# stanford-iprl-lab/nerf_shared

Measured on AMD Instinct MI355X. Metric: rays_per_sec, higher is better.
Workload: dtype bf16; 1 GPU; lego_halfres_400x400_64c+128f_viewdirs_8x256_chunk4096; entry=Renderer.render(c2w=pose, retraw=False), chunk=4096, N_samples=64, N_importance=128, weights=random-init seeds 0/10, parallelism=single GPU

## Files before the change

### nerf_shared_amd/csrc/capi.hip

```cpp
#include <hip/hip_runtime.h>

#include <atomic>
#include <cmath>

#include <cstdio>
#include <cstring>
#include <mutex>
#include <utility>
#include <new>
#include <string>
#include <vector>

#include "kernels.h"
#include "program.h"

using namespace na;

namespace {
thread_local std::string g_err;

std::string lds_msg(const char *what, size_t bytes) {
    return std::string(what) + ": the per-ray scratch needs " + std::to_string(bytes) + " bytes of LDS per workgroup, the CU has " +
           std::to_string(LDS_LIMIT_BYTES) + " (fewer samples per ray)";
}
// ... 654 lines not shown
    if (Ni > 0 && !io->u && !io->t_lin_imp) return fail(NERF_AMD_EINVAL, "need u or t_lin_imp for sample_pdf");
    const nerf_amd_model *fm = fine ? fine : coarse;
    const int och = coarse->prog.out_ch;
    if (Ni > 0 && fm->prog.out_ch != och) return fail(NERF_AMD_EINVAL, "coarse and fine models disagree on output channels");
    if (och < 4) return fail(NERF_AMD_EINVAL, "field must output at least 4 channels");
    const bool has_vd = io->ray_ch > 8;
    if ((coarse->prog.arch.use_viewdirs != 0) != has_vd || (fm->prog.arch.use_viewdirs != 0) != has_vd)
        return fail(NERF_AMD_EINVAL, "ray batch width does not match the models' use_viewdirs");
    if (io->workspace_bytes < nerf_amd_render_rays_workspace(cfg, R, och) || !io->workspace)
        return fail(NERF_AMD_EINVAL, "workspace too small");
    p->cfg = cfg; p->coarse = coarse; p->fm = fm; p->io = io; p->R = R;
    p->Nc = Nc; p->Ni = Ni; p->Nf = Nf; p->och = och; p->has_vd = has_vd;

    char *w = static_cast<char *>(io->workspace);
    auto take = [&](size_t bytes) { float *q = reinterpret_cast<float *>(w); w += align_up(bytes); return q; };
    p->z_c = take(R * Nc * sizeof(float));
    p->raw_c = take(R * Nc * och * sizeof(float));
    p->w_c = take(R * Nc * sizeof(float));
    p->z_f = p->raw_f = nullptr;
    if (Ni > 0) {
        p->z_f = take(R * (size_t)Nf * sizeof(float));
        p->raw_f = take(R * (size_t)Nf * och * sizeof(float));
        if (io->z_vals) p->z_f = io->z_vals;
        if (io->raw) p->raw_f = io->raw;
    } else {
        if (io->z_vals) p->z_c = io->z_vals;
        if (io->raw) p->raw_c = io->raw;
        if (io->weights) p->w_c = io->weights;
    }
    return NERF_AMD_OK;
}

int stage_z(ChunkPlan &p, hipStream_t s) {
    const nerf_amd_render_io *io = p.io;
    int rc = 0;
    if (io->z_coarse) {
        if (p.Ni == 0 && io->z_vals)
            rc = hipMemcpyAsync(io->z_vals, io->z_coarse, p.R * p.Nc * sizeof(float), hipMemcpyDeviceToDevice, s) == hipSuccess
                     ? 0 : NERF_AMD_EHIP;
        else
            p.z_c = const_cast<float *>(io->z_coarse);
    } else {
        rc = launch_coarse_z(io->rays, io->ray_ch, io->t_vals, p.cfg->perturb ? io->t_rand : nullptr, p.R, p.Nc,
                             p.cfg->lindisp, p.cfg->perturb, p.z_c, s);
    }
    return rc ? fail(rc, "coarse_z launch failed") : NERF_AMD_OK;
}

int stage_field(const ChunkPlan &p, bool fine_pass, hipStream_t s) {
    MlpArgs a;
    std::memset(&a, 0, sizeof(a));
    a.rays = p.io->rays; a.ray_stride = p.io->ray_ch;
    a.viewdirs = p.has_vd ? p.io->rays + 8 : nullptr; a.vd_stride = p.io->ray_ch;
    if (!fine_pass) {
        a.z_vals = p.z_c; a.P = p.R * p.Nc; a.S = p.Nc; a.out = p.raw_c;
        return run_field(p.coarse, a, p.cfg->precision, s);
    }
    a.z_vals = p.z_f; a.P = p.R * (int64_t)p.Nf; a.S = p.Nf; a.out = p.raw_f;
    return run_field(p.fm, a, p.cfg->precision, s);
}

CompositeJob final_job(const ChunkPlan &p) {
    const nerf_amd_render_io *io = p.io;
    CompositeJob j;
    std::memset(&j, 0, sizeof(j));
    const bool two_pass = p.Ni > 0;
    j.raw = two_pass ? p.raw_f : p.raw_c; j.raw_ch = p.och; j.z = two_pass ? p.z_f : p.z_c;
    j.rays_d = io->rays + 3; j.rays_d_stride = io->ray_ch;
    j.noise = p.cfg->use_noise ? (two_pass ? io->noise1 : io->noise0) : nullptr;
    j.R = p.R; j.S = two_pass ? p.Nf : p.Nc; j.white_bkgd = p.cfg->white_bkgd;
    j.rgb = io->rgb_map; j.disp = io->disp_map; j.acc = io->acc_map; j.weights = two_pass ? io->weights : p.w_c;
    return j;
}

int stage_final(const ChunkPlan &p, hipStream_t s) {
    const CompositeJob j = final_job(p);
    int rc = launch_composite(j.raw, j.raw_ch, j.z, j.rays_d, j.rays_d_stride, j.noise, j.R, j.S, j.white_bkgd, j.rgb, j.disp,
                              j.acc, j.weights, nullptr, s);
    return rc ? fail(rc, "composite launch failed") : NERF_AMD_OK;
}

int stage_mid(const ChunkPlan &p, const ChunkPlan *prev, hipStream_t s) {
    const nerf_amd_render_io *io = p.io;
    CompositeJob cj;
    std::memset(&cj, 0, sizeof(cj));
    cj.raw = p.raw_c; cj.raw_ch = p.och; cj.z = p.z_c; cj.rays_d = io->rays + 3; cj.rays_d_stride = io->ray_ch;
    cj.noise = p.cfg->use_noise ? io->noise0 : nullptr; cj.R = p.R; cj.S = p.Nc; cj.white_bkgd = p.cfg->white_bkgd;
    cj.rgb = io->rgb0; cj.disp = io->disp0; cj.acc = io->acc0; cj.weights = nullptr;
    ResampleJob rj;
    std::memset(&rj, 0, sizeof(rj));
    rj.u = io->u; rj.t_lin = io->t_lin_imp; rj.Ni = p.Ni; rj.z_fine = p.z_f; rj.z_std = io->z_std;
    CompositeJob fj;
    if (prev) fj = final_job(*prev);
    int rc = launch_mid_stage(cj, rj, prev ? &fj : nullptr, s);
    if (rc == NERF_AMD_EINVAL && resample_lds_bytes(p.Nc, p.Ni, true) > LDS_LIMIT_BYTES)
        return fail(rc, lds_msg("render_rays (compositing + resampling)", resample_lds_bytes(p.Nc, p.Ni, true)));
    return rc ? fail(rc, "composite/resample launch failed") : NERF_AMD_OK;
}
}

extern "C" {

int nerf_amd_render_rays(const nerf_amd_render_cfg *cfg, const nerf_amd_model *coarse, const nerf_amd_model *fine,
                         const nerf_amd_render_io *io, int64_t R, void *stream) {
    if (R == 0 && cfg && coarse && io) return NERF_AMD_OK;
    ChunkPlan p;
    int rc = plan_chunk(cfg, coarse, fine, io, R, &p);
    if (rc) return rc;
    hipStream_t s = static_cast<hipStream_t>(stream);
    if ((rc = stage_z(p, s)) || (rc = stage_field(p, false, s))) return rc;
    if (p.Ni == 0) return stage_final(p, s);
    if ((rc = stage_mid(p, nullptr, s)) || (rc = stage_field(p, true, s))) return rc;
    return stage_final(p, s);
}

int nerf_amd_render_chunks(const nerf_amd_render_cfg *cfg, const nerf_amd_model *coarse, const nerf_amd_model *fine,
                           const nerf_amd_render_io *ios, const int64_t *R, int32_t n_chunks, void *stream) {
    if (n_chunks < 0 || (n_chunks > 0 && (!ios || !R))) return fail(NERF_AMD_EINVAL, "bad chunk list");
    hipStream_t s = static_cast<hipStream_t>(stream);
    std::vector<ChunkPlan> plans;
    plans.reserve(n_chunks);
    for (int i = 0; i < n_chunks; ++i) {
        if (R[i] <= 0) continue;
        ChunkPlan p;
        int rc = plan_chunk(cfg, coarse, fine, &ios[i], R[i], &p);
        if (rc) return rc;
        plans.push_back(p);
    }
    const int n = (int)plans.size();
    for (int i = 0; i + 1 < n; ++i)
        if (plans[i].io->workspace == plans[i + 1].io->workspace)
            return fail(NERF_AMD_EINVAL, "consecutive chunks must use distinct workspaces");
    int rc = 0;
    for (int k = 0; k < n && !rc; ++k) {
        ChunkPlan &p = plans[k];
        if ((rc = stage_z(p, s)) || (rc = stage_field(p, false, s))) break;
        if (p.Ni == 0) { rc = stage_final(p, s); continue; }
        if ((rc = stage_mid(p, k > 0 ? &plans[k - 1] : nullptr, s))) break;
        rc = stage_field(p, true, s);
    }
    if (!rc && n > 0 && plans[n - 1].Ni > 0) rc = stage_final(plans[n - 1], s);
    return rc;
}

}

namespace {
constexpr int64_t SUPER_CHUNK_RAYS = 32768;
constexpr int BATCH_SLOTS = 3;

struct SideLane {
    hipStream_t stream = nullptr;
    hipStream_t more[2] = {nullptr, nullptr};
    std::vector<hipEvent_t> free_events;
};
std::mutex g_lane_mu;
SideLane g_lanes[64];

}
namespace na {
namespace {
struct DeviceGuard {
    int prev = -1;
    bool switched = false;
    hipError_t err = hipSuccess;
    explicit DeviceGuard(int device) {
        err = hipGetDevice(&prev);
        if (err == hipSuccess && prev != device) {
            err = hipSetDevice(device);
            switched = err == hipSuccess;
        }
    }
    ~DeviceGuard() { if (switched) (void)hipSetDevice(prev); }
};
}

int lane_acquire(int device, int n_events, hipStream_t *side, std::vector<hipEvent_t> *events) {
    if (device < 0 || device >= 64) return fail(NERF_AMD_EINVAL, "device index out of range");
    std::lock_guard<std::mutex> lk(g_lane_mu);
    DeviceGuard guard(device);
    if (guard.err != hipSuccess) return hip_fail(guard.err, "hipSetDevice(lane device)");
    SideLane &l = g_lanes[device];
    if (!l.stream) HIP_TRY(hipStreamCreateWithFlags(&l.stream, hipStreamNonBlocking));
    *side = l.stream;
    events->clear();
    for (int i = 0; i < n_events; ++i) {
        hipEvent_t e;
        if (!l.free_events.empty()) { e = l.free_events.back(); l.free_events.pop_back(); }
        else if (hipError_t err = hipEventCreateWithFlags(&e, hipEventDisableTiming); err != hipSuccess) {
            for (hipEvent_t got : *events) l.free_events.push_back(got);
            events->clear();
            return hip_fail(err, "hipEventCreateWithFlags");
        }
        events->push_back(e);
    }
    return NERF_AMD_OK;
}
int lane_streams(int device, int n, hipStream_t *out) {
    if (device < 0 || device >= 64 || n < 1 || n > 3) return fail(NERF_AMD_EINVAL, "lane_streams: device or count out of range");
    std::lock_guard<std::mutex> lk(g_lane_mu);
    DeviceGuard guard(device);
    if (guard.err != hipSuccess) return hip_fail(guard.err, "hipSetDevice(lane device)");
    SideLane &l = g_lanes[device];
    if (!l.stream) HIP_TRY(hipStreamCreateWithFlags(&l.stream, hipStreamNonBlocking));
    out[0] = l.stream;
    for (int i = 1; i < n; ++i) {
        if (!l.more[i - 1]) HIP_TRY(hipStreamCreateWithFlags(&l.more[i - 1], hipStreamNonBlocking));
        out[i] = l.more[i - 1];
    }
    return NERF_AMD_OK;
}
void lane_release(int device, const std::vector<hipEvent_t> &events) {
    std::lock_guard<std::mutex> lk(g_lane_mu);
    for (hipEvent_t e : events) g_lanes[device].free_events.push_back(e);
}
}
namespace {

nerf_amd_render_io io_rows(const nerf_amd_render_cfg *cfg, const nerf_amd_render_io &io, int64_t r0, int och, void *ws, int64_t ws_bytes) {
    nerf_amd_render_io o = io;
    const int64_t Nc = cfg->N_samples, Ni = cfg->N_importance, Sl = Nc + Ni;
    auto f = [&](const float *p, int64_t row_floats) { return p ? p + r0 * row_floats : nullptr; };
    auto g = [&](float *p, int64_t row_floats) { return p ? p + r0 * row_floats : nullptr; };
    o.rays = f(io.rays, io.ray_ch);
    o.t_rand = f(io.t_rand, Nc); o.noise0 = f(io.noise0, Nc); o.noise1 = f(io.noise1, Sl);
    o.u = f(io.u, Ni); o.z_coarse = f(io.z_coarse, Nc);
    o.rgb_map = g(io.rgb_map, 3); o.disp_map = g(io.disp_map, 1); o.acc_map = g(io.acc_map, 1);
    o.rgb0 = g(io.rgb0, 3); o.disp0 = g(io.disp0, 1); o.acc0 = g(io.acc0, 1); o.z_std = g(io.z_std, 1);
    o.raw = g(io.raw, Sl * och); o.weights = g(io.weights, Sl); o.z_vals = g(io.z_vals, Sl);
    o.workspace = ws; o.workspace_bytes = ws_bytes;
    return o;
}

int64_t n_super_chunks(int64_t N) { return N <= SUPER_CHUNK_RAYS + SUPER_CHUNK_RAYS / 2 ? 1 : (N + SUPER_CHUNK_RAYS - 1) / SUPER_CHUNK_RAYS; }
}

extern "C" {

int64_t nerf_amd_render_batch_workspace(const nerf_amd_render_cfg *cfg, int64_t N, int32_t out_ch) {
    if (!cfg || N < 0) return -1;
    const int64_t n = n_super_chunks(N);
    const int64_t per = nerf_amd_render_rays_workspace(cfg, n == 1 ? N : SUPER_CHUNK_RAYS, out_ch);
    return per * (n < BATCH_SLOTS ? n : BATCH_SLOTS);
}

int nerf_amd_render_batch(const nerf_amd_render_cfg *cfg, const nerf_amd_model *coarse, const nerf_amd_model *fine,
                          const nerf_amd_render_io *io, int64_t N, void *stream) {
    if (!cfg || !coarse || !io || N < 0) return fail(NERF_AMD_EINVAL, "null argument");
    if (N == 0) return NERF_AMD_OK;
    const int64_t n = n_super_chunks(N);
    if (n == 1) return nerf_amd_render_rays(cfg, coarse, fine, io, N, stream);
    const int och = coarse->prog.out_ch;
    const int64_t per = nerf_amd_render_rays_workspace(cfg, SUPER_CHUNK_RAYS, och);
    const int slots = (int)(n < BATCH_SLOTS ? n : BATCH_SLOTS);
    if (!io->workspace || io->workspace_bytes < per * slots) return fail(NERF_AMD_EINVAL, "workspace too small (nerf_amd_render_batch_workspace)");
    if (!io->z_coarse && cfg->perturb && !io->t_rand) return fail(NERF_AMD_EINVAL, "perturb set but neither z_coarse nor t_rand given");

    std::vector<nerf_amd_render_io> ios((size_t)n);
    std::vector<ChunkPlan> plans((size_t)n);
    for (int64_t k = 0; k < n; ++k) {
        const int64_t r0 = k * SUPER_CHUNK_RAYS, R = (k + 1 == n) ? N - r0 : SUPER_CHUNK_RAYS;
        ios[k] = io_rows(cfg, *io, r0, och, static_cast<char *>(io->workspace) + (k % slots) * per, per);
        int rc = plan_chunk(cfg, coarse, fine, &ios[k], R, &plans[k]);
        if (rc) return rc;
    }
    hipStream_t main_s = static_cast<hipStream_t>(stream), side = nullptr;
    const int device = coarse->device;
    const bool two_pass = plans[0].Ni > 0;
    std::vector<hipEvent_t> ev;
    int rc = lane_acquire(device, (int)(3 * n + 1), &side, &ev);
    if (rc) return rc;
    hipEvent_t *ec = ev.data(), *em = ev.data() + n, *ef = ev.data() + 2 * n;
    hipEvent_t start = ev[3 * n];
    auto H = [&](hipError_t e, const char *what) { if (e != hipSuccess && !rc) rc = hip_fail(e, what); };
    H(hipEventRecord(start, main_s), "hipEventRecord");
    H(hipStreamWaitEvent(side, start, 0), "hipStreamWaitEvent");

    auto coarse_field = [&](int64_t k) {
        if (k >= slots) H(hipStreamWaitEvent(main_s, em[k - slots + (two_pass ? 1 : 0)], 0), "hipStreamWaitEvent");
        if (!rc) rc = stage_z(plans[k], main_s);
        if (!rc) rc = stage_field(plans[k], false, main_s);
        H(hipEventRecord(ec[k], main_s), "hipEventRecord");
    };
    if (two_pass) {
        hipStream_t fine_s = main_s;
        hipStream_t lanes2[2];
        if (g_variant == 44 && lane_streams(device, 2, lanes2) == NERF_AMD_OK) {
            fine_s = lanes2[1];
            H(hipStreamWaitEvent(fine_s, start, 0), "hipStreamWaitEvent");
        }
        coarse_field(0);
        for (int64_t k = 0; k < n && !rc; ++k) {
            if (k + 1 < n) coarse_field(k + 1);
            H(hipStreamWaitEvent(side, ec[k], 0), "hipStreamWaitEvent");
            if (k > 0) H(hipStreamWaitEvent(side, ef[k - 1], 0), "hipStreamWaitEvent");
            if (!rc) rc = stage_mid(plans[k], k > 0 ? &plans[k - 1] : nullptr, side);
            H(hipEventRecord(em[k], side), "hipEventRecord");
            H(hipStreamWaitEvent(fine_s, em[k], 0), "hipStreamWaitEvent");
            if (!rc) rc = stage_field(plans[k], true, fine_s);
            H(hipEventRecord(ef[k], fine_s), "hipEventRecord");
        }
        H(hipStreamWaitEvent(side, ef[n - 1], 0), "hipStreamWaitEvent");
        if (!rc) rc = stage_final(plans[n - 1], side);
    } else {
        for (int64_t k = 0; k < n && !rc; ++k) {
            coarse_field(k);
            H(hipStreamWaitEvent(side, ec[k], 0), "hipStreamWaitEvent");
            if (!rc) rc = stage_final(plans[k], side);
            H(hipEventRecord(em[k], side), "hipEventRecord");
        }
    }
    H(hipEventRecord(start, side), "hipEventRecord");
    H(hipStreamWaitEvent(main_s, start, 0), "hipStreamWaitEvent");
    lane_release(device, ev);
    return rc;
}

}

extern "C" {

int nerf_amd_set_tuning(int key, int value) {
    if (key == 0 && value >= 0 && value <= 115) { g_variant.store(value, std::memory_order_relaxed); return NERF_AMD_OK; }
    if (key == 1 && value >= 0 && value <= 1) { g_density_route.store(value, std::memory_order_relaxed); return NERF_AMD_OK; }
    return fail(NERF_AMD_EINVAL, "unknown tuning key/value");
}

int nerf_amd_profile_enable(int on) {
    std::lock_guard<std::mutex> lk(g_prof_mu);
    g_prof_on = on != 0;
    return NERF_AMD_OK;
}

int nerf_amd_profile_collect(int64_t launches[3], double total_ms[3], double total_points[3]) {
    std::lock_guard<std::mutex> lk(g_prof_mu);
    for (int c = 0; c < 3; ++c) { launches[c] = 0; total_ms[c] = 0.0; total_points[c] = 0.0; }
    for (const ProfRec &r : g_prof_recs) {
        float ms = 0.f;
        if (hipEventSynchronize(r.b) == hipSuccess && hipEventElapsedTime(&ms, r.a, r.b) == hipSuccess) {
            launches[r.cls] += 1; total_ms[r.cls] += ms; total_points[r.cls] += r.points;
        }
        g_prof_free.emplace_back(r.a, r.b);
    }
    g_prof_recs.clear();
    return NERF_AMD_OK;
}

int nerf_amd_get_rays_backward(int32_t H, int32_t W, const double *K4, int64_t pix0, int64_t n, const float *g_rays_o,
                               const float *g_rays_d, float *g_c2w, void *stream) {
    if (H < 1 || W < 1 || !K4 || pix0 < 0 || n < 0 || pix0 + n > (int64_t)H * W || !g_c2w)
        return fail(NERF_AMD_EINVAL, "bad get_rays_backward arguments");
    int rc = launch_get_rays_bwd(H, W, K4, pix0, n, g_rays_o, g_rays_d, g_c2w, static_cast<hipStream_t>(stream));
    return rc ? fail(rc, "get_rays backward launch failed") : NERF_AMD_OK;
}

int nerf_amd_img2mse(const float *x, const float *y, int64_t n, float *out, float *partials, void *stream) {
    if (n < 1 || !x || !y || !out) return fail(NERF_AMD_EINVAL, "bad img2mse arguments");
    int rc = na::launch_img2mse(x, y, n, out, partials, static_cast<hipStream_t>(stream));
    return rc ? fail(rc, rc == NERF_AMD_EINVAL ? "img2mse: n > 16384 needs the partials buffer" : "img2mse launch failed") : NERF_AMD_OK;
}

int nerf_amd_img2mse_backward(const float *x, const float *y, int64_t n, const float *g, float *gx, float *gy, void *stream) {
    if (n < 1 || !x || !y || !g) return fail(NERF_AMD_EINVAL, "bad img2mse_backward arguments");
    int rc = na::launch_img2mse_bwd(x, y, n, g, gx, gy, static_cast<hipStream_t>(stream));
    return rc ? fail(rc, "img2mse_backward launch failed") : NERF_AMD_OK;
}

int nerf_amd_assemble_rays(const float *rays_o, const float *rays_d, const float *viewdir_src, int64_t n, float near,
                           float far, float *out, void *stream) {
    if (n < 0 || (n > 0 && (!rays_o || !rays_d || !out))) return fail(NERF_AMD_EINVAL, "bad assemble_rays arguments");
    int rc = na::launch_assemble_rays(rays_o, rays_d, viewdir_src, n, near, far, out, static_cast<hipStream_t>(stream));
    return rc ? fail(rc, "assemble_rays launch failed") : NERF_AMD_OK;
}

int nerf_amd_adam_step(int32_t n, float *const *params, const float *const *grads, float *const *exp_avg,
                       float *const *exp_avg_sq, const int64_t *numel, int64_t step, double lr, double beta1,
                       double beta2, double eps, double weight_decay, void *stream) {
    if (n < 0 || step < 1 || (n > 0 && (!params || !grads || !exp_avg || !exp_avg_sq || !numel)))
        return fail(NERF_AMD_EINVAL, "bad adam arguments");
    for (int i = 0; i < n; ++i) {
        if (numel[i] < 0 || numel[i] > 0x7fffffff) return fail(NERF_AMD_EINVAL, "adam: tensor size out of range");
        if (numel[i] > 0 && (!params[i] || !grads[i] || !exp_avg[i] || !exp_avg_sq[i])) return fail(NERF_AMD_EINVAL, "adam: null tensor pointer");
    }
    const double bc1 = 1.0 - std::pow(beta1, (double)step), bc2 = 1.0 - std::pow(beta2, (double)step);
    int rc = na::launch_adam(n, params, grads, exp_avg, exp_avg_sq, numel, (float)(lr / bc1), beta1, beta2,
                             (float)eps, (float)weight_decay, (float)std::sqrt(bc2), static_cast<hipStream_t>(stream));
    return rc ? fail(rc, "adam launch failed") : NERF_AMD_OK;
}

int nerf_amd_adam_step_device(int32_t n, float *const *params, const float *const *grads, float *const *exp_avg,
                              float *const *exp_avg_sq, const int64_t *numel, int64_t *step_dev, const double *lr_dev, double beta1,
                              double beta2, double eps, double weight_decay, float *scalars_dev, void *stream) {
    if (n < 0 || !step_dev || !lr_dev || !scalars_dev || (n > 0 && (!params || !grads || !exp_avg || !exp_avg_sq || !numel)))
        return fail(NERF_AMD_EINVAL, "bad adam arguments");
    if (n > 64) return fail(NERF_AMD_EINVAL, "adam (device scalars): at most 64 tensors per call (one count advance per call)");
    for (int i = 0; i < n; ++i) {
        if (numel[i] < 0 || numel[i] > 0x7fffffff) return fail(NERF_AMD_EINVAL, "adam: tensor size out of range");
        if (numel[i] > 0 && (!params[i] || !grads[i] || !exp_avg[i] || !exp_avg_sq[i])) return fail(NERF_AMD_EINVAL, "adam: null tensor pointer");
    }
    int rc = na::launch_adam(n, params, grads, exp_avg, exp_avg_sq, numel, 0.0f, beta1, beta2, (float)eps, (float)weight_decay, 1.0f,
                             static_cast<hipStream_t>(stream), step_dev, lr_dev, scalars_dev);
    return rc ? fail(rc, "adam launch failed") : NERF_AMD_OK;
}

int nerf_amd_to8b(const float *x, int64_t n, uint8_t *out, void *stream) {
    if (n < 0 || (n > 0 && (!x || !out))) return fail(NERF_AMD_EINVAL, "bad to8b arguments");
    if ((reinterpret_cast<uintptr_t>(x) & 15) || (reinterpret_cast<uintptr_t>(out) & 3))
        return fail(NERF_AMD_EINVAL, "to8b: x must be 16-byte and out 4-byte aligned");
    int rc = launch_to8b(x, n, out, static_cast<hipStream_t>(stream));
    return rc ? fail(rc, "to8b launch failed") : NERF_AMD_OK;
}

int nerf_amd_rays_at_pixels(int32_t H, int32_t W, const double *K4, const float *c2w, int32_t c2w_row_stride, const int32_t *pix,
                            int64_t n, float *rays_o, float *rays_d, void *stream) {
    if (H < 1 || W < 1 || !K4 || !c2w || c2w_row_stride < 4 || n < 0 || (n > 0 && (!pix || !rays_o || !rays_d)))
        return fail(NERF_AMD_EINVAL, "bad rays_at_pixels arguments");
    int rc = launch_rays_at_pixels(K4, c2w, c2w_row_stride, pix, n, rays_o, rays_d, static_cast<hipStream_t>(stream));
    return rc ? fail(rc, "rays_at_pixels launch failed") : NERF_AMD_OK;
}

int nerf_amd_rays_at_pixels_backward(int32_t H, int32_t W, const double *K4, const int32_t *pix, int64_t n, const float *g_rays_o,
                                     const float *g_rays_d, float *g_c2w, float *partials, void *stream) {
    if (H < 1 || W < 1 || !K4 || n < 0 || (n > 0 && !pix) || !g_c2w) return fail(NERF_AMD_EINVAL, "bad rays_at_pixels_backward arguments");
    int rc = launch_rays_at_pixels_bwd(K4, pix, n, g_rays_o, g_rays_d, g_c2w, partials, static_cast<hipStream_t>(stream));
    return rc ? fail(rc, rc == NERF_AMD_EINVAL ? "rays_at_pixels_backward: n > 16384 needs the partials buffer (256 * 12 floats)"
                                               : "rays_at_pixels_backward launch failed") : NERF_AMD_OK;
}

int nerf_amd_se3_transform(const float *w, const float *v, const float *theta, const float *x, float *T, void *stream) {
    if (!w || !v || !theta || !x || !T) return fail(NERF_AMD_EINVAL, "bad se3_transform arguments");
    int rc = launch_se3_transform(w, v, theta, x, T, static_cast<hipStream_t>(stream));
    return rc ? fail(rc, "se3_transform launch failed") : NERF_AMD_OK;
}

int nerf_amd_se3_transform_backward(const float *w, const float *v, const float *theta, const float *x, const float *g_T, float *g_w,
                                    float *g_v, float *g_theta, void *stream) {
    if (!w || !v || !theta || !x || !g_T || !g_w || !g_v || !g_theta) return fail(NERF_AMD_EINVAL, "bad se3_transform_backward arguments");
    int rc = launch_se3_transform_bwd(w, v, theta, x, g_T, g_w, g_v, g_theta, static_cast<hipStream_t>(stream));
    return rc ? fail(rc, "se3_transform_backward launch failed") : NERF_AMD_OK;
}

int nerf_amd_make_rays(int32_t H, int32_t W, const double *K4, const float *c2w, const float *c2w_static,
                       int64_t pix0, int64_t n, float near, float far, int use_viewdirs, int ndc,
                       float *rays_out, void *stream) {
    if (H < 1 || W < 1 || !K4 || !c2w || pix0 < 0 || n < 0 || pix0 + n > (int64_t)H * W || (n > 0 && !rays_out))
        return fail(NERF_AMD_EINVAL, "bad make_rays arguments");
    int rc = launch_make_rays(H, W, K4, c2w, c2w_static, pix0, n, near, far, use_viewdirs, ndc, rays_out,
                              static_cast<hipStream_t>(stream));
    return rc ? fail(rc, "make_rays launch failed") : NERF_AMD_OK;
}

}
```

### nerf_shared_amd/render_utils.py

```python
import ctypes
import os

import numpy as np
import torch

from . import _lib, utils
from . import nerf as nerf_mod
from ._lib import lib
from .nerf import NeRF

DEBUG = False

_KEYS_MAIN = ('rgb_map', 'disp_map', 'acc_map')


def _workspace(device, nbytes):
    return torch.empty(max(int(nbytes), 1), dtype=torch.uint8, device=device)


_side_streams = {}
_draw_streams = {}


def _draw_stream(device):
# ... 31 lines not shown

class _Raw2OutputsFn(torch.autograd.Function):

    @staticmethod
    def forward(ctx, raw, z, d, noise, white):
        dev = raw.device
        R, S, ch = raw.shape
        f = dict(device=dev, dtype=torch.float32)
        rgb_map, disp_map, acc_map = torch.empty(R, 3, **f), torch.empty(R, **f), torch.empty(R, **f)
        weights, depth_map = torch.empty(R, S, **f), torch.empty(R, **f)
        with torch.cuda.device(dev):
            _lib.check(lib.nerf_amd_raw2outputs(raw.data_ptr(), ch, z.data_ptr(), d.data_ptr(), d.stride(0), _lib.ptr(noise),
                                                R, S, int(white), rgb_map.data_ptr(), disp_map.data_ptr(),
                                                acc_map.data_ptr(), weights.data_ptr(), depth_map.data_ptr(),
                                                _lib.stream_of(dev)), "nerf_amd_raw2outputs")
        ctx.save_for_backward(raw, z, d, noise if noise is not None else torch.empty(0, device=dev))
        ctx.white = white
        ctx.set_materialize_grads(False)
        return rgb_map, disp_map, acc_map, weights, depth_map

    @staticmethod
    def backward(ctx, g_rgb, g_disp, g_acc, g_w, g_depth):
        raw, z, d, noise = ctx.saved_tensors
        noise = noise if noise.numel() else None
        R, S, ch = raw.shape
        g = [None if t is None else t.contiguous().float() for t in (g_rgb, g_disp, g_acc, g_depth, g_w)]
        g_raw = torch.empty_like(raw)
        g_d = torch.empty(R, 3, device=raw.device, dtype=torch.float32) if ctx.needs_input_grad[2] else None
        with torch.cuda.device(raw.device):
            _lib.check(lib.nerf_amd_raw2outputs_backward(raw.data_ptr(), ch, z.data_ptr(), d.data_ptr(), d.stride(0),
                                                         _lib.ptr(noise), R, S, int(ctx.white), _lib.ptr(g[0]),
                                                         _lib.ptr(g[1]), _lib.ptr(g[2]), _lib.ptr(g[3]), _lib.ptr(g[4]),
                                                         g_raw.data_ptr(), _lib.ptr(g_d), _lib.stream_of(raw.device)),
                       "nerf_amd_raw2outputs_backward")
        return g_raw, None, g_d, None, None


class Renderer(torch.nn.Module):
    def __init__(self, perturb=True, N_importance=128, N_samples=64, use_viewdirs=True,
                 white_bkgd=True, raw_noise_std=0.0, ndc=False, lindisp=False,
                 near=0.0, far=1.0):
        super(Renderer, self).__init__()
        self.perturb = perturb
        self.N_importance = N_importance
        self.N_samples = N_samples
        self.use_viewdirs = use_viewdirs
        self.white_bkgd = white_bkgd
        self.raw_noise_std = raw_noise_std
        self.ndc = ndc
        self.lindisp = lindisp
        self.near = near
        self.far = far
        if os.environ.get("NERF_AMD_QUIET") != "1":
            print(self.__dict__)

    def render_from_pose(self, H, W, K, chunk, c2w, coarse_model, fine_model, retraw=True):
        rgb, disp, acc, extras = self.render(
            H, W, K, coarse_model, fine_model, chunk=chunk, c2w=c2w, retraw=retraw)
        return rgb, disp, acc, extras

    def render_from_rays(self, H, W, K, chunk, rays, coarse_model, fine_model, retraw=True):
        rgb, disp, acc, extras = self.render(H, W, K, coarse_model, fine_model,
                                             chunk=chunk, rays=rays, retraw=retraw)
        return rgb, disp, acc, extras

    def render_path(self):
        pass

    def _cfg(self, precision):
        cfg = _lib.RenderCfg()
        cfg.N_samples, cfg.N_importance = int(self.N_samples), int(self.N_importance)
        cfg.perturb = int(self.perturb > 0.)
        cfg.lindisp, cfg.white_bkgd = int(bool(self.lindisp)), int(bool(self.white_bkgd))
        cfg.use_noise = int(self.raw_noise_std > 0.)
        cfg.precision = precision
        return cfg

    @staticmethod
    def _check_model(m, name):
        if not isinstance(m, NeRF):
            raise TypeError("%s must be a nerf_shared_amd.nerf.NeRF or a reference-style NeRF module (got %s)" % (name, type(m).__name__))

    def _handles(self, dev, coarse_model, fine_model):
        self._check_model(coarse_model, "coarse_model")
        if fine_model is not None:
            self._check_model(fine_model, "fine_model")
        use_fine = fine_model is not None and int(self.N_importance) > 0
        coarse_model._ensure_handle(dev)
        if use_fine:
            fine_model._ensure_handle(dev)
        prec = coarse_model._precision_code()
        if use_fine and fine_model._precision_code() != prec:
            prec = _lib.PREC_FP32
        hc = coarse_model._model_handle(dev, _lib.COPY_OF[prec])
        hf = fine_model._model_handle(dev, _lib.COPY_OF[prec]) if use_fine else None
        return hc, hf, self._cfg(prec), lib.nerf_amd_model_out_ch(hc)

    def _chunk_io(self, rays, cfg, out_ch, outs, pytest, ws=None, z_pre=None, t_rand_out=None):
        R, dev = rays.shape[0], rays.device
        Nc, Ni = int(self.N_samples), int(self.N_importance)
        Nf = Nc + Ni
        t_rand = noise0 = noise1 = u = None
        if self.perturb > 0.:
            if t_rand_out is not None:
                t_rand_out.uniform_()
            else:
                t_rand = _pytest_uniform([R, Nc], dev) if pytest else torch.rand([R, Nc], device=dev)
        if self.raw_noise_std > 0.:
            noise0 = (_pytest_uniform([R, Nc], dev) if pytest else torch.randn([R, Nc], device=dev)) * self.raw_noise_std
        t_lin = None
        if Ni > 0:
            det = (self.perturb == 0.)
            if pytest:
                np.random.seed(0)
                if det:
                    u = np.broadcast_to(np.linspace(0., 1., Ni), [R, Ni])
                else:
                    u = np.random.rand(R, Ni)
                u = torch.Tensor(np.ascontiguousarray(u)).to(dev)
            elif det:
                t_lin = _linspace01(Ni, dev)
            else:
                u = torch.rand([R, Ni], device=dev)
            if self.raw_noise_std > 0.:
                noise1 = (_pytest_uniform([R, Nf], dev) if pytest else torch.randn([R, Nf], device=dev)) * self.raw_noise_std

        io = _lib.RenderIO()
        io.rays, io.ray_ch = rays.data_ptr(), rays.shape[1]
        io.t_vals = _linspace01(Nc, dev).data_ptr()
        io.t_rand, io.noise0, io.noise1 = _lib.ptr(t_rand), _lib.ptr(noise0), _lib.ptr(noise1)
        io.u, io.t_lin_imp = _lib.ptr(u), _lib.ptr(t_lin)
        io.z_coarse = _lib.ptr(z_pre)
        for k in ('rgb_map', 'disp_map', 'acc_map', 'rgb0', 'disp0', 'acc0', 'z_std', 'raw', 'weights', 'z_vals'):
            setattr(io, k, _lib.ptr(outs.get(k)))
        nbytes = lib.nerf_amd_render_rays_workspace(cfg, R, out_ch)
        if ws is None or ws.numel() < nbytes:
            ws = _workspace(dev, nbytes)
        io.workspace, io.workspace_bytes = ws.data_ptr(), ws.numel()
        return io, (rays, t_rand, noise0, noise1, u, z_pre, ws)

    def _launch(self, rays, coarse_model, fine_model, outs, retraw, retweights, pytest):
        dev = rays.device
        hc, hf, cfg, out_ch = self._handles(dev, coarse_model, fine_model)
        io, keep = self._chunk_io(rays, cfg, out_ch, outs, pytest)
        with torch.cuda.device(dev):
            _lib.check(lib.nerf_amd_render_rays(cfg, hc, hf, io, rays.shape[0], _lib.stream_of(dev)), "nerf_amd_render_rays")
        return keep

    def _launch_batch(self, rays, starts, chunk, coarse_model, fine_model, full):
        dev = rays.device
        hc, hf, cfg, out_ch = self._handles(dev, coarse_model, fine_model)
        N, Nc, Ni = rays.shape[0], int(self.N_samples), int(self.N_importance)
        f = dict(device=dev, dtype=torch.float32)
        z_all = torch.empty(N, Nc, **f)
        noisy = self.raw_noise_std > 0.
        t_all = n0_all = n1_all = u_all = None
        if self.perturb > 0. or noisy:
            cur, ds = torch.cuda.current_stream(dev), _draw_stream(dev)
            with torch.cuda.stream(ds):
                t_all = torch.empty(N, Nc, **f) if self.perturb > 0. else None
                n0_all = torch.empty(N, Nc, **f) if noisy else None
                n1_all = torch.empty(N, Nc + Ni, **f) if (noisy and Ni > 0) else None
                u_all = torch.empty(N, Ni, **f) if (Ni > 0 and self.perturb > 0.) else None
                for i in starts:
                    if t_all is not None:
                        t_all[i:i + chunk].uniform_()
                    if n0_all is not None:
                        n0_all[i:i + chunk].normal_()
                    if u_all is not None:
                        u_all[i:i + chunk].uniform_()
                    if n1_all is not None:
                        n1_all[i:i + chunk].normal_()
                if noisy:
                    n0_all.mul_(self.raw_noise_std)
                    if n1_all is not None:
                        n1_all.mul_(self.raw_noise_std)
                drawn = torch.cuda.Event()
                drawn.record(ds)
            cur.wait_event(drawn)
            for t in (t_all, n0_all, n1_all, u_all):
                if t is not None:
                    t.record_stream(cur)
        io = _lib.RenderIO()
        io.rays, io.ray_ch = rays.data_ptr(), rays.shape[1]
        io.t_vals = _linspace01(Nc, dev).data_ptr()
        io.t_rand, io.noise0, io.noise1, io.u = _lib.ptr(t_all), _lib.ptr(n0_all), _lib.ptr(n1_all), _lib.ptr(u_all)
        io.t_lin_imp = _linspace01(Ni, dev).data_ptr() if (Ni > 0 and u_all is None) else None
        io.z_coarse = z_all.data_ptr()
        for k in ('rgb_map', 'disp_map', 'acc_map', 'rgb0', 'disp0', 'acc0', 'z_std', 'raw', 'weights', 'z_vals'):
            setattr(io, k, _lib.ptr(full.get(k)))
        ws = _workspace(dev, lib.nerf_amd_render_batch_workspace(cfg, N, out_ch))
        io.workspace, io.workspace_bytes = ws.data_ptr(), ws.numel()
        with torch.cuda.device(dev):
            _lib.check(lib.nerf_amd_coarse_z(rays.data_ptr(), rays.shape[1], _linspace01(Nc, dev).data_ptr(),
                                             _lib.ptr(t_all), N, Nc, int(bool(self.lindisp)), int(self.perturb > 0.),
                                             z_all.data_ptr(), _lib.stream_of(dev)), "nerf_amd_coarse_z")
            _lib.check(lib.nerf_amd_render_batch(cfg, hc, hf, io, N, _lib.stream_of(dev)), "nerf_amd_render_batch")
        return (rays, z_all, t_all, n0_all, n1_all, u_all, ws)

    def _launch_chunks(self, rays, starts, chunk, coarse_model, fine_model, full):
        dev = rays.device
        hc, hf, cfg, out_ch = self._handles(dev, coarse_model, fine_model)
        n, N, Nc = len(starts), rays.shape[0], int(self.N_samples)
        ios = (_lib.RenderIO * n)()
        counts = (ctypes.c_int64 * n)()
        keep = []
        z_all = torch.empty(N, Nc, device=dev, dtype=torch.float32)
        t_all = torch.empty(N, Nc, device=dev, dtype=torch.float32) if self.perturb > 0. else None
        nbytes = lib.nerf_amd_render_rays_workspace(cfg, min(chunk, N), out_ch)
        wss = [_workspace(dev, nbytes), _workspace(dev, nbytes)]
        for j, i in enumerate(starts):
            part = {k: v[i:i + chunk] for k, v in full.items()}
            r = rays[i:i + chunk]
            ios[j], alive = self._chunk_io(r, cfg, out_ch, part, False, wss[j % 2], z_all[i:i + chunk],
                                           None if t_all is None else t_all[i:i + chunk])
            counts[j] = r.shape[0]
            keep.append(alive)
        with torch.cuda.device(dev):
            _lib.check(lib.nerf_amd_coarse_z(rays.data_ptr(), rays.shape[1], _linspace01(Nc, dev).data_ptr(),
                                             _lib.ptr(t_all), N, Nc, int(bool(self.lindisp)), int(self.perturb > 0.),
                                             z_all.data_ptr(), _lib.stream_of(dev)), "nerf_amd_coarse_z")
            _lib.check(lib.nerf_amd_render_chunks(cfg, hc, hf, ios, counts, n, _lib.stream_of(dev)), "nerf_amd_render_chunks")
        return keep

    def _draws(self, R, dev, pytest):
        Nc, Ni = int(self.N_samples), int(self.N_importance)
        t_rand = noise0 = noise1 = u = t_lin = None
        if self.perturb > 0.:
            t_rand = _pytest_uniform([R, Nc], dev) if pytest else torch.rand([R, Nc], device=dev)
        if self.raw_noise_std > 0.:
            noise0 = (_pytest_uniform([R, Nc], dev) if pytest else torch.randn([R, Nc], device=dev)) * self.raw_noise_std
        if Ni > 0:
            det = (self.perturb == 0.)
            if pytest:
                np.random.seed(0)
                un = np.broadcast_to(np.linspace(0., 1., Ni), [R, Ni]) if det else np.random.rand(R, Ni)
                u = torch.Tensor(np.ascontiguousarray(un)).to(dev)
            elif det:
                t_lin = _linspace01(Ni, dev)
            else:
                u = torch.rand([R, Ni], device=dev)
            if self.raw_noise_std > 0.:
                noise1 = (_pytest_uniform([R, Nc + Ni], dev) if pytest else torch.randn([R, Nc + Ni], device=dev)) * self.raw_noise_std
        return t_rand, noise0, noise1, u, t_lin

    def _render_rays_train(self, rays, coarse_model, fine_model, retraw, retweights, pytest):
        R, dev = rays.shape[0], rays.device
        Nc, Ni = int(self.N_samples), int(self.N_importance)
        t_rand, noise0, noise1, u, t_lin = self._draws(R, dev, pytest)
        f = dict(device=dev, dtype=torch.float32)
        stream = _lib.stream_of(dev)
        z = torch.empty(R, Nc, **f)
        with torch.cuda.device(dev):
            _lib.check(lib.nerf_amd_coarse_z(rays.data_ptr(), rays.shape[1], _linspace01(Nc, dev).data_ptr(), _lib.ptr(t_rand),
                                             R, Nc, int(bool(self.lindisp)), int(self.perturb > 0.), z.data_ptr(), stream),
                       "nerf_amd_coarse_z")
        rays_d = rays[:, 3:6]

        def field(net, zz):
            if net._grad_request(dev, rays)[0] == "train":
                return net.forward_rays(rays, zz)
            with torch.no_grad():
                pts = rays[:, None, 0:3] + rays[:, None, 3:6] * zz[:, :, None]
                return net.forward(pts, rays[:, 8:11] if rays.shape[1] > 8 else None)

        raw = field(coarse_model, z)
        rgb, disp, acc, weights, _ = _Raw2OutputsFn.apply(raw, z, rays_d, noise0, bool(self.white_bkgd))
        ret = {}
        if Ni > 0:
            rgb0, disp0, acc0 = rgb, disp, acc
            z_f, z_std = torch.empty(R, Nc + Ni, **f), torch.empty(R, **f)
            w_c = weights.detach()
            with torch.cuda.device(dev):
                _lib.check(lib.nerf_amd_resample(z.data_ptr(), w_c.data_ptr(), _lib.ptr(u), _lib.ptr(t_lin), R, Nc, Ni,
                                                 z_f.data_ptr(), z_std.data_ptr(), stream), "nerf_amd_resample")
            z = z_f
            net = coarse_model if fine_model is None else fine_model
            raw = field(net, z)
            rgb, disp, acc, weights, _ = _Raw2OutputsFn.apply(raw, z, rays_d, noise1, bool(self.white_bkgd))
        ret.update(rgb_map=rgb, disp_map=disp, acc_map=acc)
        if retraw:
            ret['raw'] = raw
        if retweights:
            ret['weights'] = weights if z.shape[1] > 1 else weights[:, :0]
            ret['z_vals'] = z
        if Ni > 0:
            ret.update(rgb0=rgb0, disp0=disp0, acc0=acc0, z_std=z_std)
        return ret

    def _alloc_outputs(self, R, dev, out_ch, retraw, retweights):
        Ni = int(self.N_importance)
        S_last = int(self.N_samples) + Ni
        f = dict(device=dev, dtype=torch.float32)
        outs = {'rgb_map': torch.empty(R, 3, **f), 'disp_map': torch.empty(R, **f), 'acc_map': torch.empty(R, **f)}
        if retraw:
            outs['raw'] = torch.empty(R, S_last, out_ch, **f)
        if retweights:
            outs['weights'] = torch.empty(R, S_last, **f)
            outs['z_vals'] = torch.empty(R, S_last, **f)
        if Ni > 0:
            outs['rgb0'] = torch.empty(R, 3, **f)
            outs['disp0'] = torch.empty(R, **f)
            outs['acc0'] = torch.empty(R, **f)
            outs['z_std'] = torch.empty(R, **f)
        return outs

    def _grad_mode(self, coarse_model, fine_model, rays):
        reqs = [coarse_model._grad_request(rays.device, rays)]
        if fine_model is not None and self.N_importance > 0:
            reqs.append(fine_model._grad_request(rays.device, rays))
        for m, d in reqs:
            if m == "defer":
                return m, d
        return ("train", None) if any(m == "train" for m, _ in reqs) else ("none", None)

    def render_rays(self, ray_batch, coarse_model, fine_model, retraw=False, retweights=False,
                    verbose=False, pytest=False):
        _lib.require_device(ray_batch, "ray_batch")
        coarse_model, fine_model = nerf_mod.adopt(coarse_model), nerf_mod.adopt(fine_model)
        rays = ray_batch.detach().contiguous().float()
        if rays.dim() != 2 or rays.shape[1] not in (8, 11):
            raise _lib.NerfAmdError("ray_batch must be [N, 8] or [N, 11], got %s" % (tuple(ray_batch.shape),))
        self._check_model(coarse_model, "coarse_model")
        if fine_model is not None:
            self._check_model(fine_model, "fine_model")
        mode, deferred = self._grad_mode(coarse_model, fine_model, ray_batch) if rays.shape[0] > 0 else ("none", None)
        if mode == "train":
            live = ray_batch.contiguous().float() if (torch.is_grad_enabled() and ray_batch.requires_grad) else rays
            return self._render_rays_train(live, coarse_model, fine_model, retraw, retweights, pytest)
        out_ch = 4 if coarse_model.use_viewdirs else coarse_model.output_ch
        outs = self._alloc_outputs(rays.shape[0], rays.device, out_ch, retraw, retweights)
        self._launch(rays, coarse_model, fine_model, outs, retraw, retweights, pytest)
        if retweights and outs['weights'].shape[1] == 1:
            outs['weights'] = outs['weights'][:, :0]
        ret = nerf_mod.attach_deferred_grad(outs, deferred)
        if DEBUG:
            for k in ret:
                if torch.isnan(ret[k]).any() or torch.isinf(ret[k]).any():
                    print(f"! [Numerical Error] {k} contains nan or inf.")
        return ret

    pipeline_batch = True
    fuse_chunk_launches = True
    overlap_chunks = False

    def render_batch(self, coarse_model, fine_model, rays_flat, chunk=1024 * 32, retraw=False):
        _lib.require_device(rays_flat, "rays_flat")
        coarse_model, fine_model = nerf_mod.adopt(coarse_model), nerf_mod.adopt(fine_model)
        rays = rays_flat.detach().contiguous().float()
        self._check_model(coarse_model, "coarse_model")
        N, dev = rays.shape[0], rays.device
        out_ch = 4 if coarse_model.use_viewdirs else coarse_model.output_ch
        starts = list(range(0, N, chunk))
        mode, deferred = self._grad_mode(coarse_model, fine_model, rays_flat) if N > 0 else ("none", None)
        if mode == "defer":
            with torch.no_grad():
                plain = self.render_batch(coarse_model, fine_model, rays_flat, chunk, retraw)
            return nerf_mod.attach_deferred_grad(plain, deferred)
        if mode == "train":
            live = rays_flat if (torch.is_grad_enabled() and rays_flat.requires_grad) else rays
            parts = {}
            for i in starts:
                r = self.render_rays(live[i:i + chunk], coarse_model, fine_model, retraw)
                for k, v in r.items():
                    parts.setdefault(k, []).append(v)
            return {k: (v[0] if len(v) == 1 else torch.cat(v, 0)) for k, v in parts.items()}
        full = self._alloc_outputs(N, dev, out_ch, retraw, False)
        if self.pipeline_batch and N > 0 and (len(starts) > 1 or N > 49152):
            self._launch_batch(rays, starts, chunk, coarse_model, fine_model, full)
            return full
        if not (self.overlap_chunks and len(starts) > 1):
            if len(starts) > 1 and self.fuse_chunk_launches:
                self._launch_chunks(rays, starts, chunk, coarse_model, fine_model, full)
                return full
            for i in starts:
                part = {k: v[i:i + chunk] for k, v in full.items()}
                self._launch(rays[i:i + chunk], coarse_model, fine_model, part, retraw, False, False)
            return full
        _linspace01(int(self.N_samples), dev)
        if self.N_importance > 0:
            _linspace01(int(self.N_importance), dev)
        self._handles(dev, coarse_model, fine_model)
        cur = torch.cuda.current_stream(dev)
        ready = torch.cuda.Event()
        ready.record(cur)
        side = _chunk_streams(dev)
        for s in side:
            s.wait_event(ready)
        for n, i in enumerate(starts):
            with torch.cuda.stream(side[n % len(side)]):
                part = {k: v[i:i + chunk] for k, v in full.items()}
                self._launch(rays[i:i + chunk], coarse_model, fine_model, part, retraw, False, False)
        for s in side:
            cur.wait_stream(s)
        for v in full.values():
            v.record_stream(side[0]); v.record_stream(side[1])
        return full

    def render(self, H, W, K, coarse_model, fine_model, chunk=1024 * 32, rays=None, retraw=True,
               c2w=None, c2w_staticcam=None):
        coarse_model, fine_model = nerf_mod.adopt(coarse_model), nerf_mod.adopt(fine_model)
        if c2w is not None:
            dev = next(coarse_model.parameters()).device
            if not dev.type == 'cuda':
                raise _lib.NerfAmdError("models are on %s; nerf_shared_amd runs on ROCm devices only" % dev)
            batch = utils.make_ray_batch(H, W, K, c2w, self.near, self.far, self.use_viewdirs, self.ndc,
                                         c2w_staticcam=c2w_staticcam, device=dev)
            sh = (H, W, 3)
        else:
            rays_o, rays_d = rays
            _lib.require_device(rays_d, "rays")
            sh = rays_d.shape
            tracked = torch.is_grad_enabled() and (rays_o.requires_grad or rays_d.requires_grad)
            if (not tracked and c2w_staticcam is None and rays_o.dtype == torch.float32 and rays_d.dtype == torch.float32
                    and rays_o.is_cuda and rays_o.shape == rays_d.shape and rays_d.numel() > 0):
                src = rays_d.detach().reshape(-1, 3).contiguous() if self.use_viewdirs else None
                o, d = rays_o.detach(), rays_d.detach()
                if self.ndc:
                    o, d = utils.ndc_rays(H, W, K[0][0], 1., o, d)
                o, d = o.reshape(-1, 3).contiguous(), d.reshape(-1, 3).contiguous()
                batch = torch.empty(o.shape[0], 11 if self.use_viewdirs else 8, device=o.device, dtype=torch.float32)
                with torch.cuda.device(o.device):
                    _lib.check(lib.nerf_amd_assemble_rays(o.data_ptr(), d.data_ptr(), _lib.ptr(src), o.shape[0], float(self.near),
                                                          float(self.far), batch.data_ptr(), _lib.stream_of(o.device)),
                               "nerf_amd_assemble_rays")
            else:
                viewdirs = None
                if self.use_viewdirs:
                    viewdirs = rays_d
                    if c2w_staticcam is not None:
                        rays_o, rays_d = utils.get_rays(H, W, K, c2w_staticcam)
                    viewdirs = viewdirs / torch.norm(viewdirs, dim=-1, keepdim=True)
                    viewdirs = torch.reshape(viewdirs, [-1, 3]).float()
                sh = rays_d.shape
                if self.ndc:
                    rays_o, rays_d = utils.ndc_rays(H, W, K[0][0], 1., rays_o, rays_d)
                rays_o = torch.reshape(rays_o, [-1, 3]).float()
                rays_d = torch.reshape(rays_d, [-1, 3]).float()
                near, far = self.near * torch.ones_like(rays_d[..., :1]), self.far * torch.ones_like(rays_d[..., :1])
                batch = torch.cat([rays_o, rays_d, near, far], -1)
                if self.use_viewdirs:
                    batch = torch.cat([batch, viewdirs], -1)

        all_ret = self.render_batch(coarse_model, fine_model, batch, chunk, retraw)
        for k in all_ret:
            k_sh = list(sh[:-1]) + list(all_ret[k].shape[1:])
            all_ret[k] = torch.reshape(all_ret[k], k_sh)

        ret_list = [all_ret[k] for k in _KEYS_MAIN]
        ret_dict = {k: all_ret[k] for k in all_ret if k not in _KEYS_MAIN}
        return ret_list + [ret_dict]

    def raw2outputs(self, raw, z_vals, rays_d, pytest=False):
        _lib.require_device(raw, "raw")
        dev = raw.device
        raw_c = raw.detach().contiguous().float()
        if raw_c.dim() != 3 or raw_c.shape[-1] < 4:
            raise _lib.NerfAmdError("raw must be [num_rays, num_samples, >=4]")
        R, S, ch = raw_c.shape
        z = z_vals.detach().contiguous().float()
        d = rays_d.detach().contiguous().float()
        noise = None
        if self.raw_noise_std > 0.:
            noise = (_pytest_uniform([R, S], dev) if pytest else torch.randn([R, S], device=dev)) * self.raw_noise_std
        if torch.is_grad_enabled() and (raw.requires_grad or rays_d.requires_grad):
            out = _Raw2OutputsFn.apply(raw.contiguous().float(), z, rays_d.contiguous().float(), noise, bool(self.white_bkgd))
        else:
            with torch.no_grad():
                out = _Raw2OutputsFn.apply(raw_c, z, d, noise, bool(self.white_bkgd))
        if S == 1:
            out = (out[0], out[1], out[2], out[3][:, :0], out[4])
        return out

    def render_from_batch_poses(self, H, W, K, chunk, batch_c2w, coarse_model, fine_model,
                                retraw, save_directory, b_combine_as_video=False, tb_writer=None, io_workers=4):
        from . import image_io
        os.makedirs(save_directory, exist_ok=True)
        keep_float = b_combine_as_video or tb_writer is not None
        rgbs, frames = [], []
        writer = image_io.AsyncImageWriter(io_workers) if io_workers > 0 else None
        copy_stream = None
        try:
            with torch.no_grad():
                for i, c2w in enumerate(batch_c2w):
                    rgb, _, _, _ = self.render_from_pose(H, W, K, chunk=chunk, c2w=c2w,
                                                         coarse_model=coarse_model, fine_model=fine_model)
                    rgb8 = utils.to8b(rgb)
                    filename = os.path.join(save_directory, '{:03d}.png'.format(i))
                    if keep_float:
                        rgbs.append(rgb.cpu().numpy())
                    if writer is None:
                        frames.append(rgb8.cpu().numpy())
                        image_io.write_png(filename, frames[-1])
                        continue
                    dev = rgb8.device
# ... 31 lines not shown
```

Baseline: 5.093 million rays/s.

## Move coarse z sampling onto low-priority side stream and deepen batch pipeline

Coarse z-value generation moves from a separate Python-side pre-pass into the batch library, where it runs ahead on the side stream per slot and is joined to the main stream through events. The side stream becomes a lowest-priority stream by default. The mid stage for chunk k+1 is now issued before the fine field of chunk k, which lets coarse work run one chunk further ahead. The intent is to remove the serial z pre-pass and hide the small z, mid and final stages behind the large field kernels. The cost is more events and cross-stream dependencies, plus a risk that the low-priority stream delays work on the critical path.

```diff
diff --git a/nerf_shared_amd/csrc/capi.hip b/nerf_shared_amd/csrc/capi.hip
--- a/nerf_shared_amd/csrc/capi.hip
+++ b/nerf_shared_amd/csrc/capi.hip
@@ -830,6 +830,7 @@
 struct SideLane {
     hipStream_t stream = nullptr;
     hipStream_t more[2] = {nullptr, nullptr};
+    hipStream_t low = nullptr;
     std::vector<hipEvent_t> free_events;
 };
 std::mutex g_lane_mu;
@@ -888,6 +889,20 @@
     }
     return NERF_AMD_OK;
 }
+int lane_low_priority(int device, hipStream_t *out) {
+    if (device < 0 || device >= 64) return fail(NERF_AMD_EINVAL, "device index out of range");
+    std::lock_guard<std::mutex> lk(g_lane_mu);
+    DeviceGuard guard(device);
+    if (guard.err != hipSuccess) return hip_fail(guard.err, "hipSetDevice(lane device)");
+    SideLane &l = g_lanes[device];
+    if (!l.low) {
+        int least = 0, greatest = 0;
+        HIP_TRY(hipDeviceGetStreamPriorityRange(&least, &greatest));
+        HIP_TRY(hipStreamCreateWithPriority(&l.low, hipStreamNonBlocking, least));
+    }
+    *out = l.low;
+    return NERF_AMD_OK;
+}
 void lane_release(int device, const std::vector<hipEvent_t> &events) {
     std::lock_guard<std::mutex> lk(g_lane_mu);
     for (hipEvent_t e : events) g_lanes[device].free_events.push_back(e);
@@ -946,46 +961,84 @@
     const int device = coarse->device;
     const bool two_pass = plans[0].Ni > 0;
     std::vector<hipEvent_t> ev;
-    int rc = lane_acquire(device, (int)(3 * n + 1), &side, &ev);
+    int rc = lane_acquire(device, (int)(4 * n + 1), &side, &ev);
     if (rc) return rc;
     hipEvent_t *ec = ev.data(), *em = ev.data() + n, *ef = ev.data() + 2 * n;
-    hipEvent_t start = ev[3 * n];
+    hipEvent_t *ez = ev.data() + 3 * n;
+    hipEvent_t start = ev[4 * n];
+    const int variant = g_variant;
+    const bool pair_prev = variant == 62 || variant == 44;
+    if (variant != 63 && !pair_prev) {
+        hipStream_t low = nullptr;
+        if (na::lane_low_priority(device, &low) == NERF_AMD_OK) side = low;
+    }
     auto H = [&](hipError_t e, const char *what) { if (e != hipSuccess && !rc) rc = hip_fail(e, what); };
     H(hipEventRecord(start, main_s), "hipEventRecord");
     H(hipStreamWaitEvent(side, start, 0), "hipStreamWaitEvent");
 
+    const bool z_here = !io->z_coarse;
+    auto side_z = [&](int64_t k) {
+        if (!z_here || k >= n) return;
+        if (!rc) rc = stage_z(plans[k], side);
+        H(hipEventRecord(ez[k], side), "hipEventRecord");
+    };
+    for (int64_t k = 1; k < slots; ++k) side_z(k);
     auto coarse_field = [&](int64_t k) {
-        if (k >= slots) H(hipStreamWaitEvent(main_s, em[k - slots + (two_pass ? 1 : 0)], 0), "hipStreamWaitEvent");
-        if (!rc) rc = stage_z(plans[k], main_s);
+        if (k >= slots) H(hipStreamWaitEvent(main_s, em[k - slots + (two_pass ? (pair_prev ? 1 : 2) : 0)], 0), "hipStreamWaitEvent");
+        if (z_here && k > 0) H(hipStreamWaitEvent(main_s, ez[k], 0), "hipStreamWaitEvent");
+        else if (!rc) rc = stage_z(plans[k], main_s);
         if (!rc) rc = stage_field(plans[k], false, main_s);
         H(hipEventRecord(ec[k], main_s), "hipEventRecord");
     };
     if (two_pass) {
         hipStream_t fine_s = main_s;
         hipStream_t lanes2[2];
-        if (g_variant == 44 && lane_streams(device, 2, lanes2) == NERF_AMD_OK) {
+        if (variant == 44 && lane_streams(device, 2, lanes2) == NERF_AMD_OK) {
             fine_s = lanes2[1];
             H(hipStreamWaitEvent(fine_s, start, 0), "hipStreamWaitEvent");
         }
-        coarse_field(0);
-        for (int64_t k = 0; k < n && !rc; ++k) {
-            if (k + 1 < n) coarse_field(k + 1);
+        auto mid = [&](int64_t k, int64_t fin) {
             H(hipStreamWaitEvent(side, ec[k], 0), "hipStreamWaitEvent");
-            if (k > 0) H(hipStreamWaitEvent(side, ef[k - 1], 0), "hipStreamWaitEvent");
-            if (!rc) rc = stage_mid(plans[k], k > 0 ? &plans[k - 1] : nullptr, side);
+            if (fin >= 0) H(hipStreamWaitEvent(side, ef[fin], 0), "hipStreamWaitEvent");
+            if (!rc) rc = stage_mid(plans[k], fin >= 0 ? &plans[fin] : nullptr, side);
             H(hipEventRecord(em[k], side), "hipEventRecord");
+            side_z(k + slots);
+        };
+        auto fine_field = [&](int64_t k) {
             H(hipStreamWaitEvent(fine_s, em[k], 0), "hipStreamWaitEvent");
             if (!rc) rc = stage_field(plans[k], true, fine_s);
             H(hipEventRecord(ef[k], fine_s), "hipEventRecord");
+        };
+        auto fin_alone = [&](int64_t k) {
+            H(hipStreamWaitEvent(side, ef[k], 0), "hipStreamWaitEvent");
+            if (!rc) rc = stage_final(plans[k], side);
+        };
+        coarse_field(0);
+        if (pair_prev) {
+            for (int64_t k = 0; k < n && !rc; ++k) {
+                if (k + 1 < n) coarse_field(k + 1);
+                mid(k, k - 1);
+                fine_field(k);
+            }
+            fin_alone(n - 1);
+        } else {
+            mid(0, -1);
+            for (int64_t k = 0; k < n && !rc; ++k) {
+                if (k + 1 < n) {
+                    coarse_field(k + 1);
+                    mid(k + 1, k - 1);
+                }
+                fine_field(k);
+                if (k + 2 >= n) fin_alone(k);
+            }
         }
-        H(hipStreamWaitEvent(side, ef[n - 1], 0), "hipStreamWaitEvent");
-        if (!rc) rc = stage_final(plans[n - 1], side);
     } else {
         for (int64_t k = 0; k < n && !rc; ++k) {
             coarse_field(k);
             H(hipStreamWaitEvent(side, ec[k], 0), "hipStreamWaitEvent");
             if (!rc) rc = stage_final(plans[k], side);
             H(hipEventRecord(em[k], side), "hipEventRecord");
+            side_z(k + slots);
         }
     }
     H(hipEventRecord(start, side), "hipEventRecord");
diff --git a/nerf_shared_amd/render_utils.py b/nerf_shared_amd/render_utils.py
--- a/nerf_shared_amd/render_utils.py
+++ b/nerf_shared_amd/render_utils.py
@@ -207,7 +207,7 @@
         hc, hf, cfg, out_ch = self._handles(dev, coarse_model, fine_model)
         N, Nc, Ni = rays.shape[0], int(self.N_samples), int(self.N_importance)
         f = dict(device=dev, dtype=torch.float32)
-        z_all = torch.empty(N, Nc, **f)
+        z_all = None if self.batch_z_in_library else torch.empty(N, Nc, **f)
         noisy = self.raw_noise_std > 0.
         t_all = n0_all = n1_all = u_all = None
         if self.perturb > 0. or noisy:
@@ -241,15 +241,16 @@
         io.t_vals = _linspace01(Nc, dev).data_ptr()
         io.t_rand, io.noise0, io.noise1, io.u = _lib.ptr(t_all), _lib.ptr(n0_all), _lib.ptr(n1_all), _lib.ptr(u_all)
         io.t_lin_imp = _linspace01(Ni, dev).data_ptr() if (Ni > 0 and u_all is None) else None
-        io.z_coarse = z_all.data_ptr()
+        io.z_coarse = _lib.ptr(z_all)
         for k in ('rgb_map', 'disp_map', 'acc_map', 'rgb0', 'disp0', 'acc0', 'z_std', 'raw', 'weights', 'z_vals'):
             setattr(io, k, _lib.ptr(full.get(k)))
         ws = _workspace(dev, lib.nerf_amd_render_batch_workspace(cfg, N, out_ch))
         io.workspace, io.workspace_bytes = ws.data_ptr(), ws.numel()
         with torch.cuda.device(dev):
-            _lib.check(lib.nerf_amd_coarse_z(rays.data_ptr(), rays.shape[1], _linspace01(Nc, dev).data_ptr(),
-                                             _lib.ptr(t_all), N, Nc, int(bool(self.lindisp)), int(self.perturb > 0.),
-                                             z_all.data_ptr(), _lib.stream_of(dev)), "nerf_amd_coarse_z")
+            if z_all is not None:
+                _lib.check(lib.nerf_amd_coarse_z(rays.data_ptr(), rays.shape[1], _linspace01(Nc, dev).data_ptr(),
+                                                 _lib.ptr(t_all), N, Nc, int(bool(self.lindisp)), int(self.perturb > 0.),
+                                                 z_all.data_ptr(), _lib.stream_of(dev)), "nerf_amd_coarse_z")
             _lib.check(lib.nerf_amd_render_batch(cfg, hc, hf, io, N, _lib.stream_of(dev)), "nerf_amd_render_batch")
         return (rays, z_all, t_all, n0_all, n1_all, u_all, ws)
 
@@ -396,6 +397,7 @@
         return ret
 
     pipeline_batch = True
+    batch_z_in_library = True
     fuse_chunk_launches = True
     overlap_chunks = False
 
```

Result: no change. 5.091 million rays/s (-0.0%).
